# facebookresearch/actionmesh

Measured on NVIDIA H100. Metric: denoiser_steps_per_sec, higher is better.
Workload: dtype bf16

## Files before the change

actionmesh_b200/csrc/gemm.cu:

```cuda
#include <atomic>
#include <cstdlib>
#include "common.cuh"
#include "ptx.cuh"
#include "../../include/actionmesh_b200.h"

namespace amb {

constexpr int BM = 128;
constexpr int BK = 64;
constexpr int GEMM_THREADS = 384;
constexpr int CLUSTER = 2;
constexpr int GROUP_M = 8;
constexpr int EPI_BATCH = 4;

struct GemmParams {
  int M, N, K;
  int k_split_blocks;
  void* C;
  long long ldc;
  int c_fp32;
  const float* bias;
  const void* residual;
  long long ldr;
  int res_fp32;
  int act;
  const float* col_scale;
  int grp_rows, grp_stride, row_off;
  int norm_cols, norm_seg;
  const float* norm_w0;
  const float* norm_w1;
  float norm_eps;
  int rope_cols;
  const float* rope_cos;
  const float* rope_sin;
  int rope_rows_per_pos;
  void* C2;
  long long ldc2;
};

__device__ __forceinline__ float gelu_erf(float x) {
  const float ax = fabsf(x);
  float t;
  asm("rcp.approx.ftz.f32 %0, %1;" : "=f"(t) : "f"(fmaf(0.3275911f * 0.70710678118654752440f, ax, 1.0f)));
  float p = fmaf(t, 1.061405429f, -1.453152027f);
  p = fmaf(p, t, 1.421413741f);
  p = fmaf(p, t, -0.284496736f);
  p = fmaf(p, t, 0.254829592f);
  const float e = ex2_approx(ax * ax * (-0.5f * 1.4426950408889634f));
  const float q = 0.5f * (p * t) * e;
  return x * (x >= 0.0f ? 1.0f - q : q);
}

template <int BN>
struct GemmSmem {
  static constexpr int STAGES = BN == 128 ? 6 : 8;
  static constexpr int A_BYTES = BM * BK * 2;
  static constexpr int B_BYTES = BN * BK * 2;
  static constexpr int STAGE_BYTES = A_BYTES + B_BYTES;
  static constexpr int BAR_OFFSET = STAGES * STAGE_BYTES;
  static constexpr int TOTAL = BAR_OFFSET + 2 * STAGES * 8 + 1024;
};

__device__ __forceinline__ void store2(void* C, int c_fp32, long long off, float v0, float v1) {
  if (c_fp32) *reinterpret_cast<float2*>(reinterpret_cast<float*>(C) + off) = make_float2(v0, v1);
  else *reinterpret_cast<uint32_t*>(reinterpret_cast<__nv_bfloat16*>(C) + off) = pack_bf16(v0, v1);
}
__device__ __forceinline__ float2 load2(const void* R, int r_fp32, long long off) {
  if (r_fp32) return *reinterpret_cast<const float2*>(reinterpret_cast<const float*>(R) + off);
  return unpack_bf16(*reinterpret_cast<const uint32_t*>(reinterpret_cast<const __nv_bfloat16*>(R) + off));
}

__device__ __forceinline__ void finish_pair(const GemmParams& p, float v0, float v1, float2 r, long long drow, int col,
                                            bool valid) {
  if (p.bias) {
    const float2 b = __ldg(reinterpret_cast<const float2*>(p.bias + col));
    v0 += b.x; v1 += b.y;
  }
  if (p.act == 1) {
    v0 = gelu_erf(v0);
    v1 = gelu_erf(v1);
  }
  if (p.col_scale) {
    const float2 s = __ldg(reinterpret_cast<const float2*>(p.col_scale + col));
    v0 *= s.x; v1 *= s.y;
  }
  if (!valid) return;
  if (p.residual) { v0 += r.x; v1 += r.y; }
  store2(p.C, p.c_fp32, drow * p.ldc + col, v0, v1);
  if (p.C2) store2(p.C2, 0, drow * p.ldc2 + col, v0, v1);
}

template <int BN>
__device__ __forceinline__ void epilogue_tile(const GemmParams& p, const float* acc, int n0, int r0) {
  const int q = threadIdx.x & 3;
  long long drow[2];
  bool valid[2];
  int row[2] = {r0, r0 + 8};
#pragma unroll
  for (int h = 0; h < 2; ++h) {
    valid[h] = row[h] < p.M;
    drow[h] = row[h];
    if (p.grp_rows > 0) drow[h] = (long long)(row[h] / p.grp_rows) * p.grp_stride + (row[h] % p.grp_rows) + p.row_off;
  }
  if constexpr (BN == 128) {
    const bool do_norm = n0 < p.norm_cols, do_rope = n0 < p.rope_cols;
    if (do_norm || do_rope) {
      float rs[2] = {1.0f, 1.0f};
      float2 nw[16];
      if (do_norm) {
        const float* w = (n0 < p.norm_seg) ? p.norm_w0 : p.norm_w1;
#pragma unroll
        for (int i = 0; i < 16; ++i) nw[i] = __ldg(reinterpret_cast<const float2*>(w + 8 * i + 2 * q));
        float ss0 = 0.f, ss1 = 0.f;
#pragma unroll
        for (int i = 0; i < 16; ++i) {
          ss0 += acc[4 * i] * acc[4 * i] + acc[4 * i + 1] * acc[4 * i + 1];
          ss1 += acc[4 * i + 2] * acc[4 * i + 2] + acc[4 * i + 3] * acc[4 * i + 3];
        }
        ss0 += __shfl_xor_sync(0xffffffffu, ss0, 1);
        ss1 += __shfl_xor_sync(0xffffffffu, ss1, 1);
        ss0 += __shfl_xor_sync(0xffffffffu, ss0, 2);
        ss1 += __shfl_xor_sync(0xffffffffu, ss1, 2);
        rs[0] = rsqrtf(ss0 * (1.0f / 128.0f) + p.norm_eps);
        rs[1] = rsqrtf(ss1 * (1.0f / 128.0f) + p.norm_eps);
      }
#pragma unroll
      for (int h = 0; h < 2; ++h) {
        float rc[16], rsn[16];
        if (do_rope) {
          const int pos = (valid[h] ? row[h] : 0) / p.rope_rows_per_pos;
          const float* cs = p.rope_cos + (long long)pos * 64;
          const float* sn = p.rope_sin + (long long)pos * 64;
#pragma unroll
          for (int i = 0; i < 16; ++i) {
            rc[i] = __ldg(cs + 4 * i + q);
            rsn[i] = __ldg(sn + 4 * i + q);
          }
        }
#pragma unroll
        for (int i = 0; i < 16; ++i) {
          const int lc = 8 * i + 2 * q;
          float v0 = acc[4 * i + 2 * h], v1 = acc[4 * i + 2 * h + 1];
          if (do_norm) {
            v0 *= rs[h] * nw[i].x;
            v1 *= rs[h] * nw[i].y;
          }
          if (do_rope) {
            const float c = rc[i], s = rsn[i];
            const float x = v0, y = v1;
            v0 = x * c - y * s;
            v1 = y * c + x * s;
          }
          if (valid[h]) store2(p.C, p.c_fp32, drow[h] * p.ldc + n0 + lc, v0, v1);
        }
      }
      return;
    }
  }
#pragma unroll
  for (int i0 = 0; i0 < BN / 8; i0 += EPI_BATCH) {
    float2 r[EPI_BATCH][2];
#pragma unroll
    for (int i = 0; i < EPI_BATCH; ++i)
#pragma unroll
      for (int h = 0; h < 2; ++h)
        r[i][h] = (p.residual && valid[h]) ? load2(p.residual, p.res_fp32, drow[h] * p.ldr + n0 + 8 * (i0 + i) + 2 * q)
                                           : make_float2(0.f, 0.f);
#pragma unroll
    for (int i = 0; i < EPI_BATCH; ++i) {
      const int col = n0 + 8 * (i0 + i) + 2 * q;
      const float* a = acc + 4 * (i0 + i);
      finish_pair(p, a[0], a[1], r[i][0], drow[0], col, valid[0]);
      finish_pair(p, a[2], a[3], r[i][1], drow[1], col, valid[1]);
    }
  }
}

template <int BN>
__device__ __forceinline__ void wgmma_tile_k16(float* acc, uint64_t adesc, uint64_t bdesc) {
  if constexpr (BN == 128) wgmma_ss_n128(acc, adesc, bdesc, 1u);
  else wgmma_ss_n64(acc, adesc, bdesc, 1u);
}

__device__ __forceinline__ void unit_tile(int u, int num_mp, int num_n, uint32_t rank, int& m0, int& nt) {
  const int band = u / (GROUP_M * num_n);
  const int first = band * GROUP_M;
  const int rows = min(GROUP_M, num_mp - first);
  const int r = u - band * GROUP_M * num_n;
  m0 = ((first + r % rows) * CLUSTER + (int)rank) * BM;
  nt = r / rows;
}

template <int BN>
__global__ void __cluster_dims__(CLUSTER, 1, 1) __launch_bounds__(GEMM_THREADS, 1)
gemm_bf16_kernel(const __grid_constant__ CUtensorMap tmA, const __grid_constant__ CUtensorMap tmA2,
                 const __grid_constant__ CUtensorMap tmB, const GemmParams p) {
  using L = GemmSmem<BN>;
  constexpr int STAGES = L::STAGES;
  constexpr int B_HALF = L::B_BYTES / CLUSTER;
  extern __shared__ uint8_t smem_raw[];
  uint8_t* smem = reinterpret_cast<uint8_t*>((reinterpret_cast<uintptr_t>(smem_raw) + 1023) & ~uintptr_t(1023));
  uint64_t* full_bar = reinterpret_cast<uint64_t*>(smem + L::BAR_OFFSET);
  uint64_t* empty_bar = full_bar + STAGES;

  const int wg = __shfl_sync(0xffffffffu, threadIdx.x >> 7, 0);
  const int warp = threadIdx.x >> 5;
  const int lane = threadIdx.x & 31;
  const uint32_t rank = cluster_ctarank();
  if (threadIdx.x == 0) {
    tma_prefetch_desc(&tmA);
    tma_prefetch_desc(&tmA2);
    tma_prefetch_desc(&tmB);
    for (int s = 0; s < STAGES; ++s) {
      mbar_init(&full_bar[s], 1);
      mbar_init(&empty_bar[s], 4 * CLUSTER);
    }
    fence_mbar_init();
  }
  cluster_sync();

  const int num_n = p.N / BN;
  const int num_mp = (p.M + CLUSTER * BM - 1) / (CLUSTER * BM);
  const int num_units = num_mp * num_n;
  const int cluster = blockIdx.x / CLUSTER, num_clusters = gridDim.x / CLUSTER;
  const int num_kb = p.K / BK;

  if (wg == 0) {
    reg_dealloc<40>();
    if (warp == 0) {
      int s = 0;
      uint32_t phase = 0;
      for (int u = cluster; u < num_units; u += num_clusters) {
        int m0, nt;
        unit_tile(u, num_mp, num_n, rank, m0, nt);
        const int n0 = nt * BN;
        for (int kb = 0; kb < num_kb; ++kb) {
          mbar_wait(&empty_bar[s], phase ^ 1);
          if (elect_one()) {
            mbar_expect_tx(&full_bar[s], L::STAGE_BYTES);
            uint8_t* sa = smem + s * L::STAGE_BYTES;
            uint8_t* sb = sa + L::A_BYTES;
            if (kb < p.k_split_blocks) tma_load_2d(sa, &tmA, &full_bar[s], kb * BK, m0, kEvictNormal);
            else tma_load_2d(sa, &tmA2, &full_bar[s], (kb - p.k_split_blocks) * BK, m0, kEvictNormal);
            tma_load_2d_multicast(sb + rank * B_HALF, &tmB, &full_bar[s], kb * BK, n0 + (int)rank * (BN / CLUSTER),
                                  (uint16_t)((1u << CLUSTER) - 1), kEvictLast);
          }
          __syncwarp();
          if (++s == STAGES) { s = 0; phase ^= 1; }
        }
      }
      for (int j = 0; j < STAGES; ++j) {
        mbar_wait(&empty_bar[s], phase ^ 1);
        if (++s == STAGES) { s = 0; phase ^= 1; }
      }
    }
  } else {
    reg_alloc<232>();
    const uint32_t my_turn = wg, other_turn = 3 - wg;
    const int n_local = (num_units - cluster + num_clusters - 1) / num_clusters;
    for (int i = wg - 1; i < n_local; i += 2) {
      int m0, nt;
      unit_tile(cluster + i * num_clusters, num_mp, num_n, rank, m0, nt);
      const int n0 = nt * BN;
      float acc[2][BN / 2];
#pragma unroll
      for (int h = 0; h < 2; ++h)
#pragma unroll
        for (int j = 0; j < BN / 2; ++j) acc[h][j] = 0.f;
      const long long g0 = (long long)i * num_kb;
      int s = (int)(g0 % STAGES), s_prev = s;
      uint32_t phase = (uint32_t)((g0 / STAGES) & 1);
      if (i > 0) named_bar_sync(my_turn, 256);
      for (int kb = 0; kb < num_kb; ++kb) {
        mbar_wait_watched(&full_bar[s], phase);
        const uint32_t a_addr = smem_u32(smem + s * L::STAGE_BYTES);
        const uint64_t adesc0 = make_desc_kmajor_sw128(a_addr);
        const uint64_t adesc1 = make_desc_kmajor_sw128(a_addr + 64 * 128);
        const uint64_t bdesc = make_desc_kmajor_sw128(a_addr + L::A_BYTES);
        wgmma_fence();
#pragma unroll
        for (int k = 0; k < BK / 16; ++k) {
          wgmma_tile_k16<BN>(acc[0], adesc0 + 2 * k, bdesc + 2 * k);
          wgmma_tile_k16<BN>(acc[1], adesc1 + 2 * k, bdesc + 2 * k);
        }
        wgmma_commit();
        wgmma_wait<1>();
        if (kb > 0) {
          __syncwarp();
          if (lane < CLUSTER) mbar_arrive_cluster(&empty_bar[s_prev], lane);
        }
        s_prev = s;
        if (++s == STAGES) { s = 0; phase ^= 1; }
      }
      if (i + 1 < n_local) named_bar_arrive(other_turn, 256);
      wgmma_wait<0>();
#pragma unroll
      for (int h = 0; h < 2; ++h)
#pragma unroll
        for (int j = 0; j < BN / 2; ++j) reg_fence(acc[h][j]);
      __syncwarp();
      if (lane < CLUSTER) mbar_arrive_cluster(&empty_bar[s_prev], lane);
      if (m0 < p.M) {
        const int r0 = m0 + (warp & 3) * 16 + (lane >> 2);
        epilogue_tile<BN>(p, acc[0], n0, r0);
        epilogue_tile<BN>(p, acc[1], n0, r0 + 64);
      }
    }
  }
  __syncwarp();
  cluster_sync();
}

static GemmParams make_params(const amb_gemm_args* a) {
  GemmParams p;
  p.M = a->m; p.N = a->n; p.K = a->k;
  p.k_split_blocks = a->a2 ? a->k_split / BK : 0x7fffffff;
  p.C = a->c; p.ldc = a->ldc; p.c_fp32 = a->c_fp32;
  p.bias = a->bias;
  p.residual = a->residual; p.ldr = a->ldr; p.res_fp32 = a->res_fp32;
  p.act = a->act;
  p.col_scale = a->col_scale;
  p.grp_rows = a->grp_rows; p.grp_stride = a->grp_stride; p.row_off = a->row_off;
  p.norm_cols = a->norm_cols; p.norm_seg = a->norm_seg;
  p.norm_w0 = a->norm_w0; p.norm_w1 = a->norm_w1 ? a->norm_w1 : a->norm_w0;
  p.norm_eps = a->norm_eps;
  p.rope_cols = a->rope_cols; p.rope_cos = a->rope_cos; p.rope_sin = a->rope_sin;
  p.rope_rows_per_pos = a->rope_rows_per_pos > 0 ? a->rope_rows_per_pos : 1;
  p.C2 = a->c2; p.ldc2 = a->ldc2;
  return p;
}

template <int BN>
static int max_active_clusters(int* out) {
  static std::atomic<int> cached[16];
  int dev = 0;
  AMB_CHECK_CUDA(cudaGetDevice(&dev));
  if (dev < 16 && cached[dev].load() > 0) {
    *out = cached[dev].load();
    return AMB_OK;
  }
  cudaLaunchConfig_t cfg = {};
  cfg.gridDim = dim3(CLUSTER * num_sms(), 1, 1);
  cfg.blockDim = dim3(GEMM_THREADS, 1, 1);
  cfg.dynamicSmemBytes = GemmSmem<BN>::TOTAL;
  int n = 0;
  AMB_CHECK_CUDA(cudaOccupancyMaxActiveClusters(&n, gemm_bf16_kernel<BN>, &cfg));
  AMB_CHECK_ARG(n > 0, "gemm: no %d-CTA cluster of %d B shared memory fits on device %d", CLUSTER, GemmSmem<BN>::TOTAL, dev);
  if (dev < 16) cached[dev].store(n);
  *out = n;
  return AMB_OK;
}

template <int BN>
static int launch_gemm(const amb_gemm_args* a, cudaStream_t stream) {
  using L = GemmSmem<BN>;
  CUtensorMap tmA, tmA2, tmB;
  const int k1 = (a->a2 != nullptr) ? a->k_split : a->k;
  {
    uint64_t dims[2] = {(uint64_t)k1, (uint64_t)a->m};
    uint64_t str[1] = {(uint64_t)a->lda * 2};
    uint32_t box[2] = {BK, BM};
    int r = encode_tmap_bf16(&tmA, a->a, 2, dims, str, box);
    if (r) return r;
  }
  if (a->a2) {
    uint64_t dims[2] = {(uint64_t)(a->k - a->k_split), (uint64_t)a->m};
    uint64_t str[1] = {(uint64_t)a->lda2 * 2};
    uint32_t box[2] = {BK, BM};
    int r = encode_tmap_bf16(&tmA2, a->a2, 2, dims, str, box);
    if (r) return r;
  } else {
    tmA2 = tmA;
  }
  {
    uint64_t dims[2] = {(uint64_t)a->k, (uint64_t)a->n};
    uint64_t str[1] = {(uint64_t)a->ldw * 2};
    uint32_t box[2] = {BK, BN / CLUSTER};
    int r = encode_tmap_bf16(&tmB, a->w, 2, dims, str, box);
    if (r) return r;
  }
  GemmParams p = make_params(a);
  auto kern = gemm_bf16_kernel<BN>;
  {
    int r = ensure_smem_optin(kern, L::TOTAL);
    if (r) return r;
  }
  int clusters = 0;
  {
    int r = max_active_clusters<BN>(&clusters);
    if (r) return r;
  }
  const long long num_mp = ((long long)a->m + CLUSTER * BM - 1) / (CLUSTER * BM);
  const long long num_units = (long long)(a->n / BN) * num_mp;
  AMB_CHECK_ARG(num_units < 0x7fffffffLL, "gemm: too many tiles (m=%d n=%d)", a->m, a->n);
  const unsigned grid = (unsigned)(CLUSTER * (num_units < clusters ? num_units : clusters));
  kern<<<grid, GEMM_THREADS, L::TOTAL, stream>>>(tmA, tmA2, tmB, p);
  AMB_CHECK_CUDA(cudaGetLastError());
  return AMB_OK;
}

}

using namespace amb;

extern "C" int amb_gemm_bf16(const amb_gemm_args* a, amb_stream_t stream) {
  AMB_CHECK_ARG(a && a->a && a->w && a->c, "gemm: null pointer");
  AMB_CHECK_ARG(a->m > 0 && a->n > 0 && a->k > 0, "gemm: bad shape m=%d n=%d k=%d", a->m, a->n, a->k);
  AMB_CHECK_ARG(a->k % BK == 0, "gemm: k=%d must be a multiple of %d", a->k, BK);
  AMB_CHECK_ARG(a->n % 64 == 0, "gemm: n=%d must be a multiple of 64", a->n);
  AMB_CHECK_ARG(a->lda % 8 == 0 && a->ldw % 8 == 0 && a->ldc % 8 == 0, "gemm: lda/ldw/ldc must be multiples of 8 elements");
  AMB_CHECK_ARG(!a->a2 || (a->k_split > 0 && a->k_split < a->k && a->k_split % BK == 0 && a->lda2 % 8 == 0),
                "gemm: bad k_split %d", a->k_split);
  AMB_CHECK_ARG(!a->residual || a->ldr % 8 == 0, "gemm: ldr must be a multiple of 8");
  AMB_CHECK_ARG(a->act == 0 || a->act == 1, "gemm: unknown activation %d", a->act);
  AMB_CHECK_ARG(!a->c2 || a->ldc2 % 8 == 0, "gemm: ldc2 must be a multiple of 8");
  if (a->norm_cols > 0 || a->rope_cols > 0) {
    AMB_CHECK_ARG(a->n % 128 == 0 && a->norm_cols % 128 == 0 && a->rope_cols % 128 == 0,
                  "gemm: head epilogue needs n, norm_cols, rope_cols multiples of 128");
    AMB_CHECK_ARG(a->norm_cols == 0 || (a->norm_w0 && a->norm_seg % 128 == 0), "gemm: norm weights / norm_seg (multiple of 128) required");
    AMB_CHECK_ARG(a->rope_cols == 0 || (a->rope_cos && a->rope_sin), "gemm: rope tables required");
    AMB_CHECK_ARG(!a->residual && a->act == 0 && !a->col_scale && !a->c2, "gemm: head epilogue excludes residual/activation/col_scale/c2");
  }
  cudaStream_t s = (cudaStream_t)stream;
  if (a->n % 128 == 0) return launch_gemm<128>(a, s);
  return launch_gemm<64>(a, s);
}
```

actionmesh_b200/csrc/ptx.cuh:

```cuda
#pragma once
#include <cstdint>
#include <cuda_runtime.h>
#include <cuda_bf16.h>

namespace amb {

__device__ __forceinline__ uint32_t smem_u32(const void* p) {
  return static_cast<uint32_t>(__cvta_generic_to_shared(p));
}
__device__ __forceinline__ uint32_t lane_id() { return threadIdx.x & 31; }

__device__ __forceinline__ bool elect_one() {
  uint32_t pred = 0;
  asm volatile(
      "{\n\t.reg .pred P;\n\t"
      "elect.sync _|P, 0xffffffff;\n\t"
      "selp.u32 %0, 1, 0, P;\n\t}\n"
      : "=r"(pred));
  return pred != 0;
}

__device__ __forceinline__ void mbar_init(uint64_t* bar, uint32_t count) {
  asm volatile("mbarrier.init.shared::cta.b64 [%0], %1;" ::"r"(smem_u32(bar)), "r"(count) : "memory");
}
__device__ __forceinline__ void fence_mbar_init() {
  asm volatile("fence.mbarrier_init.release.cluster;" ::: "memory");
}
__device__ __forceinline__ void fence_proxy_async_smem() {
  asm volatile("fence.proxy.async.shared::cta;" ::: "memory");
}
__device__ __forceinline__ void mbar_expect_tx(uint64_t* bar, uint32_t bytes) {
  asm volatile("mbarrier.arrive.expect_tx.shared::cta.b64 _, [%0], %1;" ::"r"(smem_u32(bar)), "r"(bytes)
               : "memory");
}
__device__ __forceinline__ void mbar_arrive(uint64_t* bar) {
  asm volatile("mbarrier.arrive.shared::cta.b64 _, [%0];" ::"r"(smem_u32(bar)) : "memory");
}
__device__ __forceinline__ uint32_t mbar_try_wait(uint64_t* bar, uint32_t parity) {
  uint32_t ok;
  asm volatile(
      "{\n\t.reg .pred P;\n\t"
      "mbarrier.try_wait.parity.shared::cta.b64 P, [%1], %2;\n\t"
      "selp.u32 %0, 1, 0, P;\n\t}\n"
      : "=r"(ok)
      : "r"(smem_u32(bar)), "r"(parity)
      : "memory");
  return ok;
}
__device__ __forceinline__ void mbar_arrive_cluster(uint64_t* bar, uint32_t cta) {
  asm volatile(
      "{\n\t.reg .b32 ra;\n\t"
      "mapa.shared::cluster.u32 ra, %0, %1;\n\t"
      "mbarrier.arrive.shared::cluster.b64 _, [ra];\n\t}\n"
      ::"r"(smem_u32(bar)), "r"(cta)
      : "memory");
}

__device__ __forceinline__ uint32_t cluster_ctarank() {
  uint32_t r;
  asm volatile("mov.u32 %0, %%cluster_ctarank;" : "=r"(r));
  return r;
}
__device__ __forceinline__ void cluster_sync() {
  asm volatile("barrier.cluster.arrive.release;\n\tbarrier.cluster.wait.acquire;" ::: "memory");
}
__device__ __forceinline__ uint64_t globaltimer_ns() {
  uint64_t t;
  asm volatile("mov.u64 %0, %%globaltimer;" : "=l"(t));
  return t;
}
#ifndef AMB_WAIT_TIMEOUT_NS
#define AMB_WAIT_TIMEOUT_NS 4000000000ull
#endif
#ifndef AMB_WAIT_TIMEOUT_PRINT
#define AMB_WAIT_TIMEOUT_PRINT 0
#endif
__device__ __forceinline__ void mbar_wait(uint64_t* bar, uint32_t parity) {
  if (mbar_try_wait(bar, parity)) return;
  uint64_t t0 = globaltimer_ns();
  uint32_t spins = 0;
  while (!mbar_try_wait(bar, parity)) {
    if ((++spins & 0xfff) == 0 && globaltimer_ns() - t0 > AMB_WAIT_TIMEOUT_NS) {
#if AMB_WAIT_TIMEOUT_PRINT
      printf("amb: mbarrier wait timeout block=(%d,%d,%d) thread=%d bar=%u parity=%u\n", blockIdx.x, blockIdx.y,
             blockIdx.z, threadIdx.x, smem_u32(bar), parity);
#endif
      __trap();
    }
  }
}
__device__ __forceinline__ void mbar_wait_watched(uint64_t* bar, uint32_t parity) {
  while (!mbar_try_wait(bar, parity)) {
  }
}

__device__ __forceinline__ void tma_prefetch_desc(const void* tmap) {
  asm volatile("prefetch.tensormap [%0];" ::"l"(reinterpret_cast<uint64_t>(tmap)) : "memory");
}
constexpr uint64_t kEvictNormal = 0x1000000000000000ull;
constexpr uint64_t kEvictFirst = 0x12F0000000000000ull;
constexpr uint64_t kEvictLast = 0x14F0000000000000ull;

__device__ __forceinline__ void tma_load_2d(void* dst, const void* tmap, uint64_t* bar, int c0, int c1,
                                            uint64_t hint) {
  asm volatile(
      "cp.async.bulk.tensor.2d.shared::cluster.global.mbarrier::complete_tx::bytes.L2::cache_hint"
      " [%0], [%1, {%3, %4}], [%2], %5;"
      :
      : "r"(smem_u32(dst)), "l"(reinterpret_cast<uint64_t>(tmap)), "r"(smem_u32(bar)), "r"(c0), "r"(c1), "l"(hint)
      : "memory");
}
__device__ __forceinline__ void tma_load_2d_multicast(void* dst, const void* tmap, uint64_t* bar, int c0, int c1,
                                                      uint16_t cta_mask, uint64_t hint) {
  asm volatile(
      "cp.async.bulk.tensor.2d.shared::cluster.global.mbarrier::complete_tx::bytes.multicast::cluster.L2::cache_hint"
      " [%0], [%1, {%4, %5}], [%2], %3, %6;"
      :
      : "r"(smem_u32(dst)), "l"(reinterpret_cast<uint64_t>(tmap)), "r"(smem_u32(bar)), "h"(cta_mask), "r"(c0), "r"(c1),
        "l"(hint)
      : "memory");
}
__device__ __forceinline__ void tma_load_4d(void* dst, const void* tmap, uint64_t* bar, int c0, int c1, int c2,
                                            int c3, uint64_t hint) {
  asm volatile(
      "cp.async.bulk.tensor.4d.shared::cluster.global.mbarrier::complete_tx::bytes.L2::cache_hint"
      " [%0], [%1, {%3, %4, %5, %6}], [%2], %7;"
      :
      : "r"(smem_u32(dst)), "l"(reinterpret_cast<uint64_t>(tmap)), "r"(smem_u32(bar)), "r"(c0), "r"(c1), "r"(c2),
        "r"(c3), "l"(hint)
      : "memory");
}

__device__ __forceinline__ void tma_load_5d(void* dst, const void* tmap, uint64_t* bar, int c0, int c1, int c2,
                                            int c3, int c4, uint64_t hint) {
  asm volatile(
      "cp.async.bulk.tensor.5d.shared::cluster.global.mbarrier::complete_tx::bytes.L2::cache_hint"
      " [%0], [%1, {%3, %4, %5, %6, %7}], [%2], %8;"
      :
      : "r"(smem_u32(dst)), "l"(reinterpret_cast<uint64_t>(tmap)), "r"(smem_u32(bar)), "r"(c0), "r"(c1), "r"(c2),
        "r"(c3), "r"(c4), "l"(hint)
      : "memory");
}

__device__ __forceinline__ void wgmma_fence() { asm volatile("wgmma.fence.sync.aligned;" ::: "memory"); }
__device__ __forceinline__ void wgmma_commit() { asm volatile("wgmma.commit_group.sync.aligned;" ::: "memory"); }
template <int N>
__device__ __forceinline__ void wgmma_wait() {
  asm volatile("wgmma.wait_group.sync.aligned %0;" ::"n"(N) : "memory");
}
__device__ __forceinline__ void reg_fence(float& r) { asm volatile("" : "+f"(r)::"memory"); }

__device__ __forceinline__ uint64_t make_smem_desc(uint32_t saddr, uint32_t lbo_bytes, uint32_t sbo_bytes) {
  uint64_t d = 0;
  d |= static_cast<uint64_t>((saddr & 0x3FFFF) >> 4);
  d |= static_cast<uint64_t>((lbo_bytes >> 4) & 0x3FFF) << 16;
  d |= static_cast<uint64_t>((sbo_bytes >> 4) & 0x3FFF) << 32;
  d |= 1ull << 62;
  return d;
}
__device__ __forceinline__ uint64_t make_desc_kmajor_sw128(uint32_t saddr) { return make_smem_desc(saddr, 16, 1024); }
__device__ __forceinline__ uint64_t make_desc_mnmajor_sw128(uint32_t saddr, uint32_t lbo_bytes) {
  return make_smem_desc(saddr, lbo_bytes, 1024);
}

__device__ __forceinline__ void wgmma_ss_n64(float* d, uint64_t desc_a, uint64_t desc_b, uint32_t scale_d) {
  asm volatile(
      "{\n\t.reg .pred p;\n\tsetp.ne.b32 p, %34, 0;\n\t"
      "wgmma.mma_async.sync.aligned.m64n64k16.f32.bf16.bf16 {%0, %1, %2, %3, %4, %5, %6, %7, %8, %9, %10, %11, %12, %13, %14, %15, %16, %17, %18, %19, %20, %21, %22, %23, %24, %25, %26, %27, %28, %29, %30, %31}, %32, %33, p, 1, 1, 0, 0;\n\t}\n"
      : "+f"(d[0]), "+f"(d[1]), "+f"(d[2]), "+f"(d[3]), "+f"(d[4]), "+f"(d[5]), "+f"(d[6]), "+f"(d[7]), "+f"(d[8]), "+f"(d[9]), "+f"(d[10]), "+f"(d[11]), "+f"(d[12]), "+f"(d[13]), "+f"(d[14]), "+f"(d[15]), "+f"(d[16]), "+f"(d[17]), "+f"(d[18]), "+f"(d[19]), "+f"(d[20]), "+f"(d[21]), "+f"(d[22]), "+f"(d[23]), "+f"(d[24]), "+f"(d[25]), "+f"(d[26]), "+f"(d[27]), "+f"(d[28]), "+f"(d[29]), "+f"(d[30]), "+f"(d[31])
      : "l"(desc_a), "l"(desc_b), "r"(scale_d));
}
__device__ __forceinline__ void wgmma_ss_n128(float* d, uint64_t desc_a, uint64_t desc_b, uint32_t scale_d) {
  asm volatile(
      "{\n\t.reg .pred p;\n\tsetp.ne.b32 p, %66, 0;\n\t"
      "wgmma.mma_async.sync.aligned.m64n128k16.f32.bf16.bf16 {%0, %1, %2, %3, %4, %5, %6, %7, %8, %9, %10, %11, %12, %13, %14, %15, %16, %17, %18, %19, %20, %21, %22, %23, %24, %25, %26, %27, %28, %29, %30, %31, %32, %33, %34, %35, %36, %37, %38, %39, %40, %41, %42, %43, %44, %45, %46, %47, %48, %49, %50, %51, %52, %53, %54, %55, %56, %57, %58, %59, %60, %61, %62, %63}, %64, %65, p, 1, 1, 0, 0;\n\t}\n"
      : "+f"(d[0]), "+f"(d[1]), "+f"(d[2]), "+f"(d[3]), "+f"(d[4]), "+f"(d[5]), "+f"(d[6]), "+f"(d[7]), "+f"(d[8]), "+f"(d[9]), "+f"(d[10]), "+f"(d[11]), "+f"(d[12]), "+f"(d[13]), "+f"(d[14]), "+f"(d[15]), "+f"(d[16]), "+f"(d[17]), "+f"(d[18]), "+f"(d[19]), "+f"(d[20]), "+f"(d[21]), "+f"(d[22]), "+f"(d[23]), "+f"(d[24]), "+f"(d[25]), "+f"(d[26]), "+f"(d[27]), "+f"(d[28]), "+f"(d[29]), "+f"(d[30]), "+f"(d[31]), "+f"(d[32]), "+f"(d[33]), "+f"(d[34]), "+f"(d[35]), "+f"(d[36]), "+f"(d[37]), "+f"(d[38]), "+f"(d[39]), "+f"(d[40]), "+f"(d[41]), "+f"(d[42]), "+f"(d[43]), "+f"(d[44]), "+f"(d[45]), "+f"(d[46]), "+f"(d[47]), "+f"(d[48]), "+f"(d[49]), "+f"(d[50]), "+f"(d[51]), "+f"(d[52]), "+f"(d[53]), "+f"(d[54]), "+f"(d[55]), "+f"(d[56]), "+f"(d[57]), "+f"(d[58]), "+f"(d[59]), "+f"(d[60]), "+f"(d[61]), "+f"(d[62]), "+f"(d[63])
      : "l"(desc_a), "l"(desc_b), "r"(scale_d));
}
__device__ __forceinline__ void wgmma_ss_n256(float* d, uint64_t desc_a, uint64_t desc_b, uint32_t scale_d) {
  asm volatile(
      "{\n\t.reg .pred p;\n\tsetp.ne.b32 p, %130, 0;\n\t"
      "wgmma.mma_async.sync.aligned.m64n256k16.f32.bf16.bf16 {%0, %1, %2, %3, %4, %5, %6, %7, %8, %9, %10, %11, %12, %13, %14, %15, %16, %17, %18, %19, %20, %21, %22, %23, %24, %25, %26, %27, %28, %29, %30, %31, %32, %33, %34, %35, %36, %37, %38, %39, %40, %41, %42, %43, %44, %45, %46, %47, %48, %49, %50, %51, %52, %53, %54, %55, %56, %57, %58, %59, %60, %61, %62, %63, %64, %65, %66, %67, %68, %69, %70, %71, %72, %73, %74, %75, %76, %77, %78, %79, %80, %81, %82, %83, %84, %85, %86, %87, %88, %89, %90, %91, %92, %93, %94, %95, %96, %97, %98, %99, %100, %101, %102, %103, %104, %105, %106, %107, %108, %109, %110, %111, %112, %113, %114, %115, %116, %117, %118, %119, %120, %121, %122, %123, %124, %125, %126, %127}, %128, %129, p, 1, 1, 0, 0;\n\t}\n"
      : "+f"(d[0]), "+f"(d[1]), "+f"(d[2]), "+f"(d[3]), "+f"(d[4]), "+f"(d[5]), "+f"(d[6]), "+f"(d[7]), "+f"(d[8]), "+f"(d[9]), "+f"(d[10]), "+f"(d[11]), "+f"(d[12]), "+f"(d[13]), "+f"(d[14]), "+f"(d[15]), "+f"(d[16]), "+f"(d[17]), "+f"(d[18]), "+f"(d[19]), "+f"(d[20]), "+f"(d[21]), "+f"(d[22]), "+f"(d[23]), "+f"(d[24]), "+f"(d[25]), "+f"(d[26]), "+f"(d[27]), "+f"(d[28]), "+f"(d[29]), "+f"(d[30]), "+f"(d[31]), "+f"(d[32]), "+f"(d[33]), "+f"(d[34]), "+f"(d[35]), "+f"(d[36]), "+f"(d[37]), "+f"(d[38]), "+f"(d[39]), "+f"(d[40]), "+f"(d[41]), "+f"(d[42]), "+f"(d[43]), "+f"(d[44]), "+f"(d[45]), "+f"(d[46]), "+f"(d[47]), "+f"(d[48]), "+f"(d[49]), "+f"(d[50]), "+f"(d[51]), "+f"(d[52]), "+f"(d[53]), "+f"(d[54]), "+f"(d[55]), "+f"(d[56]), "+f"(d[57]), "+f"(d[58]), "+f"(d[59]), "+f"(d[60]), "+f"(d[61]), "+f"(d[62]), "+f"(d[63]), "+f"(d[64]), "+f"(d[65]), "+f"(d[66]), "+f"(d[67]), "+f"(d[68]), "+f"(d[69]), "+f"(d[70]), "+f"(d[71]), "+f"(d[72]), "+f"(d[73]), "+f"(d[74]), "+f"(d[75]), "+f"(d[76]), "+f"(d[77]), "+f"(d[78]), "+f"(d[79]), "+f"(d[80]), "+f"(d[81]), "+f"(d[82]), "+f"(d[83]), "+f"(d[84]), "+f"(d[85]), "+f"(d[86]), "+f"(d[87]), "+f"(d[88]), "+f"(d[89]), "+f"(d[90]), "+f"(d[91]), "+f"(d[92]), "+f"(d[93]), "+f"(d[94]), "+f"(d[95]), "+f"(d[96]), "+f"(d[97]), "+f"(d[98]), "+f"(d[99]), "+f"(d[100]), "+f"(d[101]), "+f"(d[102]), "+f"(d[103]), "+f"(d[104]), "+f"(d[105]), "+f"(d[106]), "+f"(d[107]), "+f"(d[108]), "+f"(d[109]), "+f"(d[110]), "+f"(d[111]), "+f"(d[112]), "+f"(d[113]), "+f"(d[114]), "+f"(d[115]), "+f"(d[116]), "+f"(d[117]), "+f"(d[118]), "+f"(d[119]), "+f"(d[120]), "+f"(d[121]), "+f"(d[122]), "+f"(d[123]), "+f"(d[124]), "+f"(d[125]), "+f"(d[126]), "+f"(d[127])
      : "l"(desc_a), "l"(desc_b), "r"(scale_d));
}
__device__ __forceinline__ void wgmma_rs_n64_tb(float* d, const uint32_t* a, uint64_t desc_b, uint32_t scale_d) {
  asm volatile(
      "{\n\t.reg .pred p;\n\tsetp.ne.b32 p, %37, 0;\n\t"
      "wgmma.mma_async.sync.aligned.m64n64k16.f32.bf16.bf16 {%0, %1, %2, %3, %4, %5, %6, %7, %8, %9, %10, %11, %12, %13, %14, %15, %16, %17, %18, %19, %20, %21, %22, %23, %24, %25, %26, %27, %28, %29, %30, %31}, {%32, %33, %34, %35}, %36, p, 1, 1, 1;\n\t}\n"
      : "+f"(d[0]), "+f"(d[1]), "+f"(d[2]), "+f"(d[3]), "+f"(d[4]), "+f"(d[5]), "+f"(d[6]), "+f"(d[7]), "+f"(d[8]), "+f"(d[9]), "+f"(d[10]), "+f"(d[11]), "+f"(d[12]), "+f"(d[13]), "+f"(d[14]), "+f"(d[15]), "+f"(d[16]), "+f"(d[17]), "+f"(d[18]), "+f"(d[19]), "+f"(d[20]), "+f"(d[21]), "+f"(d[22]), "+f"(d[23]), "+f"(d[24]), "+f"(d[25]), "+f"(d[26]), "+f"(d[27]), "+f"(d[28]), "+f"(d[29]), "+f"(d[30]), "+f"(d[31])
      : "r"(a[0]), "r"(a[1]), "r"(a[2]), "r"(a[3]), "l"(desc_b), "r"(scale_d));
}
__device__ __forceinline__ void wgmma_rs_n128_tb(float* d, const uint32_t* a, uint64_t desc_b, uint32_t scale_d) {
  asm volatile(
      "{\n\t.reg .pred p;\n\tsetp.ne.b32 p, %69, 0;\n\t"
      "wgmma.mma_async.sync.aligned.m64n128k16.f32.bf16.bf16 {%0, %1, %2, %3, %4, %5, %6, %7, %8, %9, %10, %11, %12, %13, %14, %15, %16, %17, %18, %19, %20, %21, %22, %23, %24, %25, %26, %27, %28, %29, %30, %31, %32, %33, %34, %35, %36, %37, %38, %39, %40, %41, %42, %43, %44, %45, %46, %47, %48, %49, %50, %51, %52, %53, %54, %55, %56, %57, %58, %59, %60, %61, %62, %63}, {%64, %65, %66, %67}, %68, p, 1, 1, 1;\n\t}\n"
      : "+f"(d[0]), "+f"(d[1]), "+f"(d[2]), "+f"(d[3]), "+f"(d[4]), "+f"(d[5]), "+f"(d[6]), "+f"(d[7]), "+f"(d[8]), "+f"(d[9]), "+f"(d[10]), "+f"(d[11]), "+f"(d[12]), "+f"(d[13]), "+f"(d[14]), "+f"(d[15]), "+f"(d[16]), "+f"(d[17]), "+f"(d[18]), "+f"(d[19]), "+f"(d[20]), "+f"(d[21]), "+f"(d[22]), "+f"(d[23]), "+f"(d[24]), "+f"(d[25]), "+f"(d[26]), "+f"(d[27]), "+f"(d[28]), "+f"(d[29]), "+f"(d[30]), "+f"(d[31]), "+f"(d[32]), "+f"(d[33]), "+f"(d[34]), "+f"(d[35]), "+f"(d[36]), "+f"(d[37]), "+f"(d[38]), "+f"(d[39]), "+f"(d[40]), "+f"(d[41]), "+f"(d[42]), "+f"(d[43]), "+f"(d[44]), "+f"(d[45]), "+f"(d[46]), "+f"(d[47]), "+f"(d[48]), "+f"(d[49]), "+f"(d[50]), "+f"(d[51]), "+f"(d[52]), "+f"(d[53]), "+f"(d[54]), "+f"(d[55]), "+f"(d[56]), "+f"(d[57]), "+f"(d[58]), "+f"(d[59]), "+f"(d[60]), "+f"(d[61]), "+f"(d[62]), "+f"(d[63])
      : "r"(a[0]), "r"(a[1]), "r"(a[2]), "r"(a[3]), "l"(desc_b), "r"(scale_d));
}

__device__ __forceinline__ void named_bar_sync(uint32_t id, uint32_t nthreads) {
  asm volatile("bar.sync %0, %1;" ::"r"(id), "r"(nthreads) : "memory");
}
__device__ __forceinline__ void named_bar_arrive(uint32_t id, uint32_t nthreads) {
  asm volatile("bar.arrive %0, %1;" ::"r"(id), "r"(nthreads) : "memory");
}

template <int N>
__device__ __forceinline__ void reg_alloc() {
  asm volatile("setmaxnreg.inc.sync.aligned.u32 %0;" ::"n"(N));
}
template <int N>
__device__ __forceinline__ void reg_dealloc() {
  asm volatile("setmaxnreg.dec.sync.aligned.u32 %0;" ::"n"(N));
}
__device__ __forceinline__ float ex2_approx(float x) {
  float y;
  asm("ex2.approx.ftz.f32 %0, %1;" : "=f"(y) : "f"(x));
  return y;
}
__device__ __forceinline__ uint32_t pack_bf16(float lo, float hi) {
  __nv_bfloat162 v = __floats2bfloat162_rn(lo, hi);
  return *reinterpret_cast<uint32_t*>(&v);
}
__device__ __forceinline__ float2 unpack_bf16(uint32_t u) {
  __nv_bfloat162 v = *reinterpret_cast<__nv_bfloat162*>(&u);
  return __bfloat1622float2(v);
}

}
```

Baseline: 1.021.

## Add cooperative 128x256 GEMM tile for large-K shapes with residual L2 prefetch

```diff
diff --git a/actionmesh_b200/csrc/gemm.cu b/actionmesh_b200/csrc/gemm.cu
--- a/actionmesh_b200/csrc/gemm.cu
+++ b/actionmesh_b200/csrc/gemm.cu
@@ -36,6 +36,7 @@
   int rope_rows_per_pos;
   void* C2;
   long long ldc2;
+  int res_row_bytes;
 };
 
 __device__ __forceinline__ float gelu_erf(float x) {
@@ -53,7 +54,7 @@
 
 template <int BN>
 struct GemmSmem {
-  static constexpr int STAGES = BN == 128 ? 6 : 8;
+  static constexpr int STAGES = BN == 256 ? 4 : BN == 128 ? 6 : 8;
   static constexpr int A_BYTES = BM * BK * 2;
   static constexpr int B_BYTES = BN * BK * 2;
   static constexpr int STAGE_BYTES = A_BYTES + B_BYTES;
@@ -90,73 +91,90 @@
   if (p.C2) store2(p.C2, 0, drow * p.ldc2 + col, v0, v1);
 }
 
-template <int BN>
-__device__ __forceinline__ void epilogue_tile(const GemmParams& p, const float* acc, int n0, int r0) {
+__device__ __forceinline__ void output_rows(const GemmParams& p, int r0, int (&row)[2], long long (&drow)[2],
+                                            bool (&valid)[2]) {
+#pragma unroll
+  for (int h = 0; h < 2; ++h) {
+    row[h] = r0 + 8 * h;
+    valid[h] = row[h] < p.M;
+    drow[h] = row[h];
+    if (p.grp_rows > 0) drow[h] = (long long)(row[h] / p.grp_rows) * p.grp_stride + (row[h] % p.grp_rows) + p.row_off;
+  }
+}
+
+__device__ __forceinline__ void epilogue_head(const GemmParams& p, const float* acc, int c0, int r0, bool do_norm,
+                                              bool do_rope) {
   const int q = threadIdx.x & 3;
   long long drow[2];
   bool valid[2];
-  int row[2] = {r0, r0 + 8};
+  int row[2];
+  output_rows(p, r0, row, drow, valid);
+  float rs[2] = {1.0f, 1.0f};
+  float2 nw[16];
+  if (do_norm) {
+    const float* w = (c0 < p.norm_seg) ? p.norm_w0 : p.norm_w1;
+#pragma unroll
+    for (int i = 0; i < 16; ++i) nw[i] = __ldg(reinterpret_cast<const float2*>(w + 8 * i + 2 * q));
+    float ss0 = 0.f, ss1 = 0.f;
+#pragma unroll
+    for (int i = 0; i < 16; ++i) {
+      ss0 += acc[4 * i] * acc[4 * i] + acc[4 * i + 1] * acc[4 * i + 1];
+      ss1 += acc[4 * i + 2] * acc[4 * i + 2] + acc[4 * i + 3] * acc[4 * i + 3];
+    }
+    ss0 += __shfl_xor_sync(0xffffffffu, ss0, 1);
+    ss1 += __shfl_xor_sync(0xffffffffu, ss1, 1);
+    ss0 += __shfl_xor_sync(0xffffffffu, ss0, 2);
+    ss1 += __shfl_xor_sync(0xffffffffu, ss1, 2);
+    rs[0] = rsqrtf(ss0 * (1.0f / 128.0f) + p.norm_eps);
+    rs[1] = rsqrtf(ss1 * (1.0f / 128.0f) + p.norm_eps);
+  }
 #pragma unroll
   for (int h = 0; h < 2; ++h) {
-    valid[h] = row[h] < p.M;
-    drow[h] = row[h];
-    if (p.grp_rows > 0) drow[h] = (long long)(row[h] / p.grp_rows) * p.grp_stride + (row[h] % p.grp_rows) + p.row_off;
-  }
+    float rc[16], rsn[16];
+    if (do_rope) {
+      const int pos = (valid[h] ? row[h] : 0) / p.rope_rows_per_pos;
+      const float* cs = p.rope_cos + (long long)pos * 64;
+      const float* sn = p.rope_sin + (long long)pos * 64;
+#pragma unroll
+      for (int i = 0; i < 16; ++i) {
+        rc[i] = __ldg(cs + 4 * i + q);
+        rsn[i] = __ldg(sn + 4 * i + q);
+      }
+    }
+#pragma unroll
+    for (int i = 0; i < 16; ++i) {
+      const int lc = 8 * i + 2 * q;
+      float v0 = acc[4 * i + 2 * h], v1 = acc[4 * i + 2 * h + 1];
+      if (do_norm) {
+        v0 *= rs[h] * nw[i].x;
+        v1 *= rs[h] * nw[i].y;
+      }
+      if (do_rope) {
+        const float c = rc[i], s = rsn[i];
+        const float x = v0, y = v1;
+        v0 = x * c - y * s;
+        v1 = y * c + x * s;
+      }
+      if (valid[h]) store2(p.C, p.c_fp32, drow[h] * p.ldc + c0 + lc, v0, v1);
+    }
+  }
+}
+
+template <int BN>
+__device__ __forceinline__ void epilogue_tile(const GemmParams& p, const float* acc, int n0, int r0) {
+  static_assert(BN <= 128, "one head at most");
+  const int q = threadIdx.x & 3;
   if constexpr (BN == 128) {
     const bool do_norm = n0 < p.norm_cols, do_rope = n0 < p.rope_cols;
     if (do_norm || do_rope) {
-      float rs[2] = {1.0f, 1.0f};
-      float2 nw[16];
-      if (do_norm) {
-        const float* w = (n0 < p.norm_seg) ? p.norm_w0 : p.norm_w1;
-#pragma unroll
-        for (int i = 0; i < 16; ++i) nw[i] = __ldg(reinterpret_cast<const float2*>(w + 8 * i + 2 * q));
-        float ss0 = 0.f, ss1 = 0.f;
-#pragma unroll
-        for (int i = 0; i < 16; ++i) {
-          ss0 += acc[4 * i] * acc[4 * i] + acc[4 * i + 1] * acc[4 * i + 1];
-          ss1 += acc[4 * i + 2] * acc[4 * i + 2] + acc[4 * i + 3] * acc[4 * i + 3];
-        }
-        ss0 += __shfl_xor_sync(0xffffffffu, ss0, 1);
-        ss1 += __shfl_xor_sync(0xffffffffu, ss1, 1);
-        ss0 += __shfl_xor_sync(0xffffffffu, ss0, 2);
-        ss1 += __shfl_xor_sync(0xffffffffu, ss1, 2);
-        rs[0] = rsqrtf(ss0 * (1.0f / 128.0f) + p.norm_eps);
-        rs[1] = rsqrtf(ss1 * (1.0f / 128.0f) + p.norm_eps);
-      }
-#pragma unroll
-      for (int h = 0; h < 2; ++h) {
-        float rc[16], rsn[16];
-        if (do_rope) {
-          const int pos = (valid[h] ? row[h] : 0) / p.rope_rows_per_pos;
-          const float* cs = p.rope_cos + (long long)pos * 64;
-          const float* sn = p.rope_sin + (long long)pos * 64;
-#pragma unroll
-          for (int i = 0; i < 16; ++i) {
-            rc[i] = __ldg(cs + 4 * i + q);
-            rsn[i] = __ldg(sn + 4 * i + q);
-          }
-        }
-#pragma unroll
-        for (int i = 0; i < 16; ++i) {
-          const int lc = 8 * i + 2 * q;
-          float v0 = acc[4 * i + 2 * h], v1 = acc[4 * i + 2 * h + 1];
-          if (do_norm) {
-            v0 *= rs[h] * nw[i].x;
-            v1 *= rs[h] * nw[i].y;
-          }
-          if (do_rope) {
-            const float c = rc[i], s = rsn[i];
-            const float x = v0, y = v1;
-            v0 = x * c - y * s;
-            v1 = y * c + x * s;
-          }
-          if (valid[h]) store2(p.C, p.c_fp32, drow[h] * p.ldc + n0 + lc, v0, v1);
-        }
-      }
+      epilogue_head(p, acc, n0, r0, do_norm, do_rope);
       return;
     }
   }
+  long long drow[2];
+  bool valid[2];
+  int row[2];
+  output_rows(p, r0, row, drow, valid);
 #pragma unroll
   for (int i0 = 0; i0 < BN / 8; i0 += EPI_BATCH) {
     float2 r[EPI_BATCH][2];
@@ -178,7 +196,8 @@
 
 template <int BN>
 __device__ __forceinline__ void wgmma_tile_k16(float* acc, uint64_t adesc, uint64_t bdesc) {
-  if constexpr (BN == 128) wgmma_ss_n128(acc, adesc, bdesc, 1u);
+  if constexpr (BN == 256) wgmma_ss_n256(acc, adesc, bdesc, 1u);
+  else if constexpr (BN == 128) wgmma_ss_n128(acc, adesc, bdesc, 1u);
   else wgmma_ss_n64(acc, adesc, bdesc, 1u);
 }
 
@@ -198,6 +217,8 @@
   using L = GemmSmem<BN>;
   constexpr int STAGES = L::STAGES;
   constexpr int B_HALF = L::B_BYTES / CLUSTER;
+  constexpr bool COOP = BN == 256;
+  constexpr int PARTS = COOP ? 1 : 2;
   extern __shared__ uint8_t smem_raw[];
   uint8_t* smem = reinterpret_cast<uint8_t*>((reinterpret_cast<uintptr_t>(smem_raw) + 1023) & ~uintptr_t(1023));
   uint64_t* full_bar = reinterpret_cast<uint64_t*>(smem + L::BAR_OFFSET);
@@ -213,7 +234,7 @@
     tma_prefetch_desc(&tmB);
     for (int s = 0; s < STAGES; ++s) {
       mbar_init(&full_bar[s], 1);
-      mbar_init(&empty_bar[s], 4 * CLUSTER);
+      mbar_init(&empty_bar[s], (COOP ? 8 : 4) * CLUSTER);
     }
     fence_mbar_init();
   }
@@ -245,6 +266,15 @@
             tma_load_2d_multicast(sb + rank * B_HALF, &tmB, &full_bar[s], kb * BK, n0 + (int)rank * (BN / CLUSTER),
                                   (uint16_t)((1u << CLUSTER) - 1), kEvictLast);
           }
+          if (COOP && p.res_row_bytes > 0 && kb == max(num_kb - 2 * STAGES, 0)) {
+#pragma unroll
+            for (int j = 0; j < BM / 32; ++j) {
+              const int r = m0 + 32 * j + lane;
+              if (r < p.M)
+                prefetch_l2_bulk(reinterpret_cast<const uint8_t*>(p.residual) + ((long long)r * p.ldr + n0) * (p.res_fp32 ? 4 : 2),
+                                 p.res_row_bytes);
+            }
+          }
           __syncwarp();
           if (++s == STAGES) { s = 0; phase ^= 1; }
         }
@@ -258,30 +288,31 @@
     reg_alloc<232>();
     const uint32_t my_turn = wg, other_turn = 3 - wg;
     const int n_local = (num_units - cluster + num_clusters - 1) / num_clusters;
-    for (int i = wg - 1; i < n_local; i += 2) {
+    for (int i = COOP ? 0 : wg - 1; i < n_local; i += COOP ? 1 : 2) {
       int m0, nt;
       unit_tile(cluster + i * num_clusters, num_mp, num_n, rank, m0, nt);
       const int n0 = nt * BN;
-      float acc[2][BN / 2];
-#pragma unroll
-      for (int h = 0; h < 2; ++h)
+      float acc[PARTS][BN / 2];
+#pragma unroll
+      for (int h = 0; h < PARTS; ++h)
 #pragma unroll
         for (int j = 0; j < BN / 2; ++j) acc[h][j] = 0.f;
       const long long g0 = (long long)i * num_kb;
       int s = (int)(g0 % STAGES), s_prev = s;
       uint32_t phase = (uint32_t)((g0 / STAGES) & 1);
-      if (i > 0) named_bar_sync(my_turn, 256);
+      const int row0 = COOP ? 64 * (wg - 1) : 0;
+      if (!COOP && i > 0) named_bar_sync(my_turn, 256);
       for (int kb = 0; kb < num_kb; ++kb) {
         mbar_wait_watched(&full_bar[s], phase);
         const uint32_t a_addr = smem_u32(smem + s * L::STAGE_BYTES);
-        const uint64_t adesc0 = make_desc_kmajor_sw128(a_addr);
-        const uint64_t adesc1 = make_desc_kmajor_sw128(a_addr + 64 * 128);
         const uint64_t bdesc = make_desc_kmajor_sw128(a_addr + L::A_BYTES);
+        const uint64_t adesc0 = make_desc_kmajor_sw128(a_addr + row0 * 128);
+        const uint64_t adesc1 = make_desc_kmajor_sw128(a_addr + (row0 + 64) * 128);
         wgmma_fence();
 #pragma unroll
         for (int k = 0; k < BK / 16; ++k) {
           wgmma_tile_k16<BN>(acc[0], adesc0 + 2 * k, bdesc + 2 * k);
-          wgmma_tile_k16<BN>(acc[1], adesc1 + 2 * k, bdesc + 2 * k);
+          if constexpr (PARTS == 2) wgmma_tile_k16<BN>(acc[1], adesc1 + 2 * k, bdesc + 2 * k);
         }
         wgmma_commit();
         wgmma_wait<1>();
@@ -292,18 +323,23 @@
         s_prev = s;
         if (++s == STAGES) { s = 0; phase ^= 1; }
       }
-      if (i + 1 < n_local) named_bar_arrive(other_turn, 256);
+      if (!COOP && i + 1 < n_local) named_bar_arrive(other_turn, 256);
       wgmma_wait<0>();
 #pragma unroll
-      for (int h = 0; h < 2; ++h)
+      for (int h = 0; h < PARTS; ++h)
 #pragma unroll
         for (int j = 0; j < BN / 2; ++j) reg_fence(acc[h][j]);
       __syncwarp();
       if (lane < CLUSTER) mbar_arrive_cluster(&empty_bar[s_prev], lane);
       if (m0 < p.M) {
-        const int r0 = m0 + (warp & 3) * 16 + (lane >> 2);
-        epilogue_tile<BN>(p, acc[0], n0, r0);
-        epilogue_tile<BN>(p, acc[1], n0, r0 + 64);
+        const int r0 = m0 + row0 + (warp & 3) * 16 + (lane >> 2);
+        if constexpr (COOP) {
+          epilogue_tile<128>(p, acc[0], n0, r0);
+          epilogue_tile<128>(p, acc[0] + 64, n0 + 128, r0);
+        } else {
+          epilogue_tile<BN>(p, acc[0], n0, r0);
+          epilogue_tile<BN>(p, acc[1], n0, r0 + 64);
+        }
       }
     }
   }
@@ -327,6 +363,7 @@
   p.rope_cols = a->rope_cols; p.rope_cos = a->rope_cos; p.rope_sin = a->rope_sin;
   p.rope_rows_per_pos = a->rope_rows_per_pos > 0 ? a->rope_rows_per_pos : 1;
   p.C2 = a->c2; p.ldc2 = a->ldc2;
+  p.res_row_bytes = 0;
   return p;
 }
 
@@ -380,6 +417,8 @@
     if (r) return r;
   }
   GemmParams p = make_params(a);
+  if (BN == 256 && a->residual && a->grp_rows <= 0 && reinterpret_cast<uintptr_t>(a->residual) % 16 == 0)
+    p.res_row_bytes = BN * (a->res_fp32 ? 4 : 2);
   auto kern = gemm_bf16_kernel<BN>;
   {
     int r = ensure_smem_optin(kern, L::TOTAL);
@@ -397,6 +436,12 @@
   kern<<<grid, GEMM_THREADS, L::TOTAL, stream>>>(tmA, tmA2, tmB, p);
   AMB_CHECK_CUDA(cudaGetLastError());
   return AMB_OK;
+}
+
+static int gemm_tile_n(const amb_gemm_args* a) {
+  if (a->n % 256 == 0 && a->k >= 4096) return 256;
+  if (a->n % 128 == 0) return 128;
+  return 64;
 }
 
 }
@@ -422,6 +467,9 @@
     AMB_CHECK_ARG(!a->residual && a->act == 0 && !a->col_scale && !a->c2, "gemm: head epilogue excludes residual/activation/col_scale/c2");
   }
   cudaStream_t s = (cudaStream_t)stream;
-  if (a->n % 128 == 0) return launch_gemm<128>(a, s);
-  return launch_gemm<64>(a, s);
-}
+  switch (gemm_tile_n(a)) {
+    case 256: return launch_gemm<256>(a, s);
+    case 128: return launch_gemm<128>(a, s);
+    default: return launch_gemm<64>(a, s);
+  }
+}
diff --git a/actionmesh_b200/csrc/ptx.cuh b/actionmesh_b200/csrc/ptx.cuh
--- a/actionmesh_b200/csrc/ptx.cuh
+++ b/actionmesh_b200/csrc/ptx.cuh
@@ -120,6 +120,9 @@
         "l"(hint)
       : "memory");
 }
+__device__ __forceinline__ void prefetch_l2_bulk(const void* src, uint32_t bytes) {
+  asm volatile("cp.async.bulk.prefetch.L2.global [%0], %1;" ::"l"(reinterpret_cast<uint64_t>(src)), "r"(bytes) : "memory");
+}
 __device__ __forceinline__ void tma_load_4d(void* dst, const void* tmap, uint64_t* bar, int c0, int c1, int c2,
                                             int c3, uint64_t hint) {
   asm volatile(
```

Measured after the change: 1.034 (median of 6 runs). +1.2%, better.
